# rgoldade/GeometricMultigridPressureSolver

Hardware: AMD Instinct MI355X
Metric: V-cycles/sec (higher is better)
Workload: dtype f32

## Files before the change

### geometricmultigridpressuresolver_amd/csrc/mgps_internal.h

```cpp
#pragma once

#include <cstdint>
#include <cstdlib>
#include <cstddef>
#include <memory>
#include <string>
#include <utility>
#include <vector>

#include "mgps.h"

namespace mgps {

constexpr int kTile = 16;

constexpr int kChunkCells = 1024;
constexpr int kWaveChunkCells = 256;
constexpr int kSegCells = 32;

void *hostBigAlloc(size_t bytes);
void hostBigFree(void *p);
void setHostBigAllocator(void *(*alloc)(size_t), void (*release)(void *));
constexpr size_t kBigBlockBytes = size_t(1) << 20;

// ... 102 lines not shown
                   bool needCoarseSolver);
void setLastGlobalError(const std::string &msg);
const char *lastGlobalError();
int apiException(const mgps_solver *h) noexcept;
extern void (*gSetHandleError)(const mgps_solver *h, const char *msg) noexcept;
#define MGPS_API_CATCH(h) catch (...) { return ::mgps::apiException(h); }

struct GridP {
    int nx, ny, nz;
    const uint8_t *lab;
    const float *wx, *wy, *wz;
    const int32_t *bnd;
    const float *rows;
    int nbnd;
    const uint8_t *bandDiag;
    int ghostLo, ghostHi;
    const int32_t *chunks;
    int nchunks, chunkCells;
    const int32_t *planeBlocks;
    int nplaneBlocks, planeZc;
    int streaming;
    int sweepPath;
    int xlo, xhi;
};
int launchActiveXRange(void *stream, const uint8_t *lab, int nx, size_t cells, int *range);

struct MixScale {
    const float *sigma = nullptr;
    float c1 = 1.f, c2 = 1.f;
};

constexpr int kPlaneRows = 16;
constexpr size_t kPlaneSweepMinPlaneBytes = size_t(4) << 20;
constexpr int kSlabEdgePlanes = kBandMaxDepth + 1;
inline int planeSweepZc(int nx, int ny, int nz)
{
    if ((nx & 3) != 0 || nx < 256 || ny < kPlaneRows) return 0;
    const size_t nbx = (nx + 255) / 256, nby = (ny + kPlaneRows - 1) / kPlaneRows;
    int zc = 32;
    while (zc > 4 && nbx * nby * size_t((nz + zc - 1) / zc) < 1024) zc >>= 1;
    return zc;
}

enum StencilOp { OP_JACOBI = 0, OP_RESIDUAL = 1, OP_APPLY = 2 };

size_t stencilSweptCells(const GridP &g);
int stencilKernelOf(const GridP &g);
// ... 216 lines not shown
```

### geometricmultigridpressuresolver_amd/csrc/mgps_kernels.hip

```cpp
#include <hip/hip_runtime.h>
#include <hip/hip_fp16.h>

#include <algorithm>
#include <cstdlib>
#include <type_traits>

#include "mgps_internal.h"

namespace mgps {

namespace {

typedef float v4f __attribute__((ext_vector_type(4)));
typedef unsigned char v4b __attribute__((ext_vector_type(4)));
__device__ __forceinline__ float4 streamLoad4(const float *p)
{
    const v4f v = __builtin_nontemporal_load(reinterpret_cast<const v4f *>(p));
    return make_float4(v.x, v.y, v.z, v.w);
}
__device__ __forceinline__ uchar4 streamLoad4(const uint8_t *p)
{
    const v4b v = __builtin_nontemporal_load(reinterpret_cast<const v4b *>(p));
    return make_uchar4(v.x, v.y, v.z, v.w);
}
// ... 112 lines not shown
    return (bid % kXcds) * per + bid / kXcds;
}

__device__ __forceinline__ bool listQuad(const int32_t *__restrict__ chunks, int chunkCells, size_t block, size_t &t, unsigned tid)
{
    if (chunkCells == kChunkCells) {
        t = size_t(chunks[block]) * 256 + tid;
        return true;
    }
    int ch;
    if (chunkCells == kWaveChunkCells) {
        ch = chunks[block * 4 + __builtin_amdgcn_readfirstlane(tid >> 6)];
        t = size_t(max(ch, 0)) * kWave + (tid & (kWave - 1));
    } else {
        const int lanes = chunkCells >> 2, shift = __ffs(lanes) - 1;
        ch = chunks[(block << (8 - shift)) + (tid >> shift)];
        t = (size_t(max(ch, 0)) << shift) + (tid & (lanes - 1));
    }
    return ch >= 0;
}
__device__ __forceinline__ bool listQuad(const int32_t *__restrict__ chunks, int chunkCells, size_t block, size_t &t) { return listQuad(chunks, chunkCells, block, t, threadIdx.x); }
__device__ __forceinline__ int listRunMask(const int32_t *chunks, int chunkCells) { return (chunks && chunkCells < kWaveChunkCells) ? (chunkCells >> 2) - 1 : kWave - 1; }

template <int OP, bool DOT, class TX, bool XZERO, bool KEEP>
__device__ __forceinline__ void stencilQuadBody(const GridP &g, TX *__restrict__ out, const TX *__restrict__ x, const float *__restrict__ b, float omega,
                                                unsigned nblocks, const int32_t *__restrict__ chunks, double *__restrict__ dotPartials, const MixScale &ms,
                                                unsigned vblock, unsigned tid, const uint32_t *__restrict__ keep)
{
    constexpr bool kMixed = !std::is_same<TX, float>::value;
    const unsigned nq = unsigned(g.nx) >> 2;
    const size_t rows = size_t(g.ny) * g.nz;
    const size_t totalQuads = size_t(nq) * rows;
    const unsigned block = remapBlock(vblock, nblocks);
    size_t t = size_t(block) * 256 + tid;
    bool valid = true;
    if (chunks) valid = listQuad(chunks, g.chunkCells, block, t, tid);
    valid = valid && t < totalQuads;
    const size_t tt = valid ? t : totalQuads - 1;
    const size_t c = tt << 2;
    const size_t sy = size_t(g.nx), sz = size_t(g.nx) * g.ny, ncells = totalQuads << 2;
    const bool nqPow2 = (nq & (nq - 1u)) == 0u;
    const int i = int((nqPow2 ? (unsigned(tt) & (nq - 1u)) : (totalQuads <= 0xffffffffull ? unsigned(tt) % nq : unsigned(tt % nq))) << 2);

    const float4 zero4 = make_float4(0.f, 0.f, 0.f, 0.f);
    const bool live = i >= g.xlo && i < g.xhi;
    valid = valid && live;
// ... 75 lines not shown
}
#define MGPS_GLOBAL_AS __attribute__((address_space(1)))
__device__ __forceinline__ float4 gLoad4(const float *base, unsigned cell)
{
    const v4f v = *(const MGPS_GLOBAL_AS v4f *)((const MGPS_GLOBAL_AS char *)base + cell * 4u);
    return make_float4(v.x, v.y, v.z, v.w);
}
__device__ __forceinline__ float4 gLoad4nt(const float *base, unsigned cell)
{
    const v4f v = __builtin_nontemporal_load((const MGPS_GLOBAL_AS v4f *)((const MGPS_GLOBAL_AS char *)base + cell * 4u));
    return make_float4(v.x, v.y, v.z, v.w);
}
__device__ __forceinline__ float gLoad1(const float *base, unsigned cell) { return *(const MGPS_GLOBAL_AS float *)((const MGPS_GLOBAL_AS char *)base + cell * 4u); }
__device__ __forceinline__ float2 gLoad2(const float *base, unsigned cell)
{
    typedef float v2f __attribute__((ext_vector_type(2)));
    const v2f v = *(const MGPS_GLOBAL_AS v2f *)((const MGPS_GLOBAL_AS char *)base + cell * 4u);
    return make_float2(v.x, v.y);
}
__device__ __forceinline__ uchar4 gLoadCodes4nt(const uint8_t *base, unsigned cell)
{
    const v4b v = __builtin_nontemporal_load((const MGPS_GLOBAL_AS v4b *)((const MGPS_GLOBAL_AS char *)base + cell));
    return make_uchar4(v.x, v.y, v.z, v.w);
}
__device__ __forceinline__ unsigned gLoadCode1(const uint8_t *base, unsigned cell) { return *((const MGPS_GLOBAL_AS uint8_t *)base + cell); }
__device__ __forceinline__ void gStore4(float *base, unsigned cell, float4 v) { *(MGPS_GLOBAL_AS v4f *)((MGPS_GLOBAL_AS char *)base + cell * 4u) = v4f{v.x, v.y, v.z, v.w}; }
__device__ __forceinline__ void gStore4nt(float *base, unsigned cell, float4 v)
{
    __builtin_nontemporal_store(v4f{v.x, v.y, v.z, v.w}, (MGPS_GLOBAL_AS v4f *)((MGPS_GLOBAL_AS char *)base + cell * 4u));
}
typedef float v2f __attribute__((ext_vector_type(2)));
__device__ __forceinline__ void gStore2(float *base, unsigned cell, float2 v) { *(MGPS_GLOBAL_AS v2f *)((MGPS_GLOBAL_AS char *)base + cell * 4u) = v2f{v.x, v.y}; }
__device__ __forceinline__ void gStore2nt(float *base, unsigned cell, float2 v)
{
    __builtin_nontemporal_store(v2f{v.x, v.y}, (MGPS_GLOBAL_AS v2f *)((MGPS_GLOBAL_AS char *)base + cell * 4u));
}

__device__ __forceinline__ float fromLeftLane(float v) { return __int_as_float(__builtin_amdgcn_update_dpp(0, __float_as_int(v), 0x138, 0xf, 0xf, false)); }
__device__ __forceinline__ float fromRightLane(float v) { return __int_as_float(__builtin_amdgcn_update_dpp(0, __float_as_int(v), 0x130, 0xf, 0xf, false)); }
typedef float v4fu __attribute__((ext_vector_type(4), aligned(4)));
__device__ __forceinline__ float4 gLoad4u(const float *base, unsigned cell)
{
    const v4fu v = *(const MGPS_GLOBAL_AS v4fu *)((const MGPS_GLOBAL_AS char *)base + cell * 4u);
    return make_float4(v.x, v.y, v.z, v.w);
}

// ... 11 lines not shown
    double dotAcc = 0.0;
    __shared__ float plane[2][(kPlaneRows + 2) * kPlanePitch];
    unsigned bid = remapBlock(blockIdx.x, gridDim.x);
    if (blocks) bid = unsigned(blocks[bid]);
    bid = __builtin_amdgcn_readfirstlane(bid);
    const unsigned bx = bid % nbx, by = (bid / nbx) % nby, bz = bid / (nbx * nby);
    const int lane = threadIdx.x & (kWave - 1), ty = threadIdx.x / kWave;
    const int i = int(bx) * 256 + lane * 4, j = int(by) * kPlaneRows + ty;
    const int ic = min(i, g.nx - 4), jc = min(j, g.ny - 1);
    const bool live = ic >= g.xlo && ic < g.xhi;
    const bool valid = i < g.nx && j < g.ny && live;
    const bool ld = live && !XZERO;
    const ptrdiff_t sz = ptrdiff_t(g.nx) * g.ny;
    const int k0 = int(bz) * zc, k1 = min(k0 + zc, g.nz);
    const int kLo = g.ghostLo ? -1 : 0, kHi = g.ghostHi ? g.nz : g.nz - 1;
    const unsigned off = unsigned(jc) * unsigned(g.nx) + unsigned(ic);
    const unsigned offYm = jc > 0 ? off - unsigned(g.nx) : off, offYp = jc < g.ny - 1 ? off + unsigned(g.nx) : off;
    auto planeOf = [&](const float *p, int k) { return scalarBase(p + ptrdiff_t(min(max(k, kLo), kHi)) * sz); };
    const bool rowTop = ty == 0, rowBot = ty == kPlaneRows - 1, colL = lane == 0, colR = lane == kWave - 1;
    const bool useHx = ld && ((colL && ic > 0) || (colR && ic + 4 < g.nx));
    const unsigned offHx = !useHx ? off : (colL ? off - 1u : off + 4u);

    const float4 zero4 = make_float4(0.f, 0.f, 0.f, 0.f);
    const uchar4 ext4 = make_uchar4(MGPS_EXTERIOR_CELL, MGPS_EXTERIOR_CELL, MGPS_EXTERIOR_CELL, MGPS_EXTERIOR_CELL);
    float *const mine0 = plane[0] + (ty + 1) * kPlanePitch + 4 + lane * 4;
    constexpr int kBufFloats = (kPlaneRows + 2) * kPlanePitch;
    *reinterpret_cast<float4 *>(mine0 + kBufFloats) = ld ? gLoad4(planeOf(x, k0 - 1), off) : zero4;
    const float *xk = XZERO ? x : planeOf(x, k0);
    float4 xc = ld ? gLoad4(xk, off) : zero4;
    float4 xp = ld ? gLoad4(planeOf(x, k0 + 1), off) : zero4;
    float4 hy = zero4;
    if (ld && rowTop) hy = gLoad4(xk, offYm);
    if (ld && rowBot) hy = gLoad4(xk, offYp);
    float hx = ld ? gLoad1(xk, offHx) : 0.f;

    int buf = 0;
    for (int k = k0; k < k1; ++k) {
        float *me = mine0 + buf * kBufFloats;
        *reinterpret_cast<float4 *>(me) = xc;
        if (rowTop) *reinterpret_cast<float4 *>(me - kPlanePitch) = hy;
        if (rowBot) *reinterpret_cast<float4 *>(me + kPlanePitch) = hy;
        if (colL) me[-1] = useHx ? hx : 0.f;
        if (colR) me[4] = useHx ? hx : 0.f;
        float4 bc = zero4;
        uchar4 lc = ext4;
        if (live) {
            if (OP != OP_APPLY) bc = gLoad4nt(scalarBase(b + ptrdiff_t(k) * sz), off);
            lc = gLoadCodes4nt(scalarBase(g.lab + ptrdiff_t(k) * sz), off);
        }
        float4 xq = zero4, hyn = hy;
        float hxn = hx;
        if (k + 1 < k1 && ld) {
            const float *xn = planeOf(x, k + 1);
            xq = gLoad4(planeOf(x, k + 2), off);
            if (rowTop) hyn = gLoad4(xn, offYm);
            if (rowBot) hyn = gLoad4(xn, offYp);
            hxn = gLoad1(xn, offHx);
        }
        __syncthreads();
        const float4 ym = *reinterpret_cast<const float4 *>(me - kPlanePitch);
        const float4 yp = *reinterpret_cast<const float4 *>(me + kPlanePitch);
        const float4 xm = *reinterpret_cast<const float4 *>(mine0 + (buf ^ 1) * kBufFloats);
        const float xs[6] = {me[-1], xc.x, xc.y, xc.z, xc.w, me[4]};
        const float yms[4] = {ym.x, ym.y, ym.z, ym.w}, yps[4] = {yp.x, yp.y, yp.z, yp.w};
        const float zms[4] = {xm.x, xm.y, xm.z, xm.w}, zps[4] = {xp.x, xp.y, xp.z, xp.w};
        const float bs[4] = {bc.x, bc.y, bc.z, bc.w};
        const unsigned ls[4] = {lc.x, lc.y, lc.z, lc.w};
        float res[4];
#pragma unroll
        for (int e = 0; e < 4; ++e) {
            const float diag = simpleDiag(ls[e]);
            const float lap = diag * xs[e + 1] - (xs[e] + xs[e + 2] + yms[e] + yps[e] + zms[e] + zps[e]);
            res[e] = simpleCell(ls[e]) ? epilogueRcp<OP>(xs[e + 1], bs[e], lap, simpleRcp(diag), omega) : inactiveValue<OP>(xs[e + 1]);
        }
        if (valid)
            gStore4nt(scalarBase(out + ptrdiff_t(k) * sz), off, make_float4(res[0], res[1], res[2], res[3]));
        if (DOT) {
#pragma unroll
            for (int e = 0; e < 4; ++e)
                if (valid && simpleCell(ls[e])) dotAcc += dotTerm<OP>(xs[e + 1], bs[e], res[e]);
        }
        xc = xp;
        xp = xq;
        hy = hyn;
        hx = hxn;
        buf ^= 1;
    }
    if (DOT) {
        __syncthreads();
// ... 14 lines not shown
    __shared__ float crow[kUpRing][kUpRows * kPlanePitch];
    unsigned bid = remapBlock(blockIdx.x, gridDim.x);
    if (blocks) bid = unsigned(blocks[bid]);
    bid = __builtin_amdgcn_readfirstlane(bid);
    const unsigned bx = bid % nbx, by = (bid / nbx) % nby, bz = bid / (nbx * nby);
    const int lane = threadIdx.x & (kWave - 1), ty = threadIdx.x / kWave;
    const int i = int(bx) * 256 + lane * 4, j = int(by) * kPlaneRows + ty;
    const int ic = min(i, g.nx - 4), jc = min(j, g.ny - 1);
    const bool live = ic >= g.xlo && ic < g.xhi;
    const bool valid = i < g.nx && j < g.ny && live;
    const ptrdiff_t sz = ptrdiff_t(g.nx) * g.ny;
    const int k0 = int(bz) * zc, k1 = min(k0 + zc, g.nz);
    const unsigned off = unsigned(jc) * unsigned(g.nx) + unsigned(ic);
    const unsigned offYm = jc > 0 ? off - unsigned(g.nx) : off, offYp = jc < g.ny - 1 ? off + unsigned(g.nx) : off;
    auto planeOf = [&](const float *p, int k) { return scalarBase(p + ptrdiff_t(min(max(k, 0), g.nz - 1)) * sz); };
    const bool rowTop = ty == 0, rowBot = ty == kPlaneRows - 1, colL = lane == 0, colR = lane == kWave - 1;
    const bool useHx = live && ((colL && ic > 0) || (colR && ic + 4 < g.nx));
    const unsigned offHx = !useHx ? off : (colL ? off - 1u : off + 4u);
    auto opq = [](unsigned v) {
        asm volatile("" : "+v"(v));
        return v;
    };
    const float4 zero4 = make_float4(0.f, 0.f, 0.f, 0.f);
    const uchar4 ext4 = make_uchar4(MGPS_EXTERIOR_CELL, MGPS_EXTERIOR_CELL, MGPS_EXTERIOR_CELL, MGPS_EXTERIOR_CELL);

    const int cnx = g.nx >> 1, cny = g.ny >> 1, cnz = g.nz >> 1;
    const ptrdiff_t csz = ptrdiff_t(cnx) * cny;
    const int tid = threadIdx.x;
    const bool stager = tid < kUpStagers;
    const int sr = tid / kUpQuads, sq = tid - sr * kUpQuads;
    const int mq = min(max(int(bx) * 64 - 1 + sq, 0), (g.nx >> 2) - 1);
    const int crw = min(max(int(by) * (kPlaneRows / 2) - 1 + sr, 0), cny - 1);
    const unsigned cOff1 = unsigned(crw) * unsigned(cnx) + unsigned(2 * mq);
    auto slotOf = [](int P) { return (P + kUpRing) % kUpRing; };
    auto cplane = [&](int P) { return scalarBase(coarse + ptrdiff_t(min(max(P, 0), cnz - 1)) * csz); };
    auto loadC = [&](const float *p) {
        const float2 c12 = gLoad2(p, opq(cOff1));
        return make_float4(gLoad1(p, opq(mq > 0 ? cOff1 - 1u : cOff1)), c12.x, c12.y, gLoad1(p, opq(2 * mq + 2 < cnx ? cOff1 + 2u : cOff1 + 1u)));
    };
    auto stageC = [&](int P, float4 c) {
        *reinterpret_cast<float4 *>(&crow[slotOf(P)][sr * kPlanePitch + 4 * sq]) =
            make_float4(lerpRef(c.x, c.y, 0.75f), lerpRef(c.y, c.z, 0.25f), lerpRef(c.y, c.z, 0.75f), lerpRef(c.z, c.w, 0.25f));
    };
    const int rowBase = 1 - int(by) * (kPlaneRows / 2);
    auto rowsAt = [&](int kk, int jj, int xi, const float *&pa, const float *&pb, float &fy, float &fz) {
        const int Pa = (kk - 1) >> 1;
        const int o = (((jj - 1) >> 1) + rowBase) * kPlanePitch + xi;
        pa = &crow[slotOf(Pa)][o];
        pb = &crow[slotOf(Pa + 1)][o];
        fy = (jj & 1) ? 0.25f : 0.75f;
        fz = (kk & 1) ? 0.25f : 0.75f;
    };
    auto trilerp = [](float a0, float a1, float b0, float b1, float fy, float fz) { return lerpRef(lerpRef(a0, a1, fy), lerpRef(b0, b1, fy), fz); };
    auto corr4 = [&](int kk, int jj, float4 v, uchar4 lc, bool act) {
        const float *pa, *pb;
        float fy, fz;
        rowsAt(kk, jj, 4 + lane * 4, pa, pb, fy, fz);
        const float4 a0 = *reinterpret_cast<const float4 *>(pa), a1 = *reinterpret_cast<const float4 *>(pa + kPlanePitch);
        const float4 ya = make_float4(lerpRef(a0.x, a1.x, fy), lerpRef(a0.y, a1.y, fy), lerpRef(a0.z, a1.z, fy), lerpRef(a0.w, a1.w, fy));
        asm volatile("" ::: "memory");
        const float4 b0 = *reinterpret_cast<const float4 *>(pb), b1 = *reinterpret_cast<const float4 *>(pb + kPlanePitch);
        const float t0 = lerpRef(ya.x, lerpRef(b0.x, b1.x, fy), fz), t1 = lerpRef(ya.y, lerpRef(b0.y, b1.y, fy), fz);
        const float t2 = lerpRef(ya.z, lerpRef(b0.z, b1.z, fy), fz), t3 = lerpRef(ya.w, lerpRef(b0.w, b1.w, fy), fz);
        return make_float4(!act || activeLabel(lc.x) ? v.x + 4.f * t0 : v.x, !act || activeLabel(lc.y) ? v.y + 4.f * t1 : v.y,
                           !act || activeLabel(lc.z) ? v.z + 4.f * t2 : v.z, !act || activeLabel(lc.w) ? v.w + 4.f * t3 : v.w);
    };
    auto corr1 = [&](int kk, int jj, float v) {
        const float *pa, *pb;
        float fy, fz;
        rowsAt(kk, jj, colL ? 3 : 4 + 256, pa, pb, fy, fz);
        return v + 4.f * trilerp(pa[0], pa[kPlanePitch], pb[0], pb[kPlanePitch], fy, fz);
    };

    {
        const float *p0 = cplane((k0 >> 1) - 1), *p1 = cplane(k0 >> 1), *p2 = cplane((k0 >> 1) + 1);
        const float4 c0 = stager ? loadC(p0) : zero4, c1 = stager ? loadC(p1) : zero4, c2 = stager ? loadC(p2) : zero4;
        if (stager) {
            stageC((k0 >> 1) - 1, c0);
            stageC(k0 >> 1, c1);
            stageC((k0 >> 1) + 1, c2);
        }
    }
    float *const mine0 = plane[0] + (ty + 1) * kPlanePitch + 4 + lane * 4;
    constexpr int kBufFloats = (kPlaneRows + 2) * kPlanePitch;
    float4 xm0 = live ? gLoad4(planeOf(x, k0 - 1), off) : zero4;
    const float *xk = planeOf(x, k0);
    float4 xc = live ? gLoad4(xk, off) : zero4;
    float4 xp = live ? gLoad4(planeOf(x, k0 + 1), off) : zero4;
    const uint8_t *lab0 = scalarBase(g.lab + ptrdiff_t(k0) * sz);
    uchar4 lc = live ? gLoadCodes4nt(lab0, off) : ext4;
    uchar4 lcn = live ? gLoadCodes4nt(scalarBase(g.lab + ptrdiff_t(k0 + 1) * sz), off) : ext4;
    float4 hy = zero4;
    if (live && rowTop) hy = gLoad4(xk, offYm);
    if (live && rowBot) hy = gLoad4(xk, offYp);
    float hx = live ? gLoad1(xk, offHx) : 0.f;
    __syncthreads();
    if (live) {
        xm0 = corr4(k0 - 1, j, xm0, lc, false);
        xc = corr4(k0, j, xc, lc, true);
    }
    *reinterpret_cast<float4 *>(mine0 + kBufFloats) = xm0;

    int buf = 0;
    for (int k = k0; k < k1; ++k) {
        float *me = mine0 + buf * kBufFloats;
        if (live) {
            if (rowTop) hy = corr4(k, j - 1, hy, lc, false);
            if (rowBot) hy = corr4(k, j + 1, hy, lc, false);
            if (useHx) hx = corr1(k, j, hx);
            xp = corr4(k + 1, j, xp, lcn, k + 1 < k1);
        }
        *reinterpret_cast<float4 *>(me) = xc;
        if (rowTop) *reinterpret_cast<float4 *>(me - kPlanePitch) = hy;
        if (rowBot) *reinterpret_cast<float4 *>(me + kPlanePitch) = hy;
        if (colL) me[-1] = useHx ? hx : 0.f;
        if (colR) me[4] = useHx ? hx : 0.f;
        float4 bc = zero4;
        uchar4 lcq = ext4;
        const float *bk = scalarBase(b + ptrdiff_t(k) * sz);
        const uint8_t *labq = scalarBase(g.lab + ptrdiff_t(min(k + 2, g.nz - 1)) * sz);
        if (live) {
            bc = gLoad4nt(bk, opq(off));
            if (k + 2 < k1) lcq = gLoadCodes4nt(labq, opq(off));
        }
        float4 xq = zero4, hyn = hy;
        float hxn = hx;
        if (k + 1 < k1 && live) {
            const float *xn = planeOf(x, k + 1);
            xq = gLoad4(planeOf(x, k + 2), opq(off));
            if (rowTop) hyn = gLoad4(xn, opq(offYm));
            if (rowBot) hyn = gLoad4(xn, opq(offYp));
            hxn = gLoad1(xn, opq(offHx));
        }
        const bool stageNext = !(k & 1) && k + 2 < k1;
        const float *pn = cplane((k >> 1) + 2);
        float4 cnext = zero4;
        if (stageNext && stager) cnext = loadC(pn);
        __syncthreads();
        if (stageNext && stager) stageC((k >> 1) + 2, cnext);
        const float4 ym = *reinterpret_cast<const float4 *>(me - kPlanePitch);
        const float4 yp = *reinterpret_cast<const float4 *>(me + kPlanePitch);
        const float4 xm = *reinterpret_cast<const float4 *>(mine0 + (buf ^ 1) * kBufFloats);
        const float xs[6] = {me[-1], xc.x, xc.y, xc.z, xc.w, me[4]};
        const float yms[4] = {ym.x, ym.y, ym.z, ym.w}, yps[4] = {yp.x, yp.y, yp.z, yp.w};
        const float zms[4] = {xm.x, xm.y, xm.z, xm.w}, zps[4] = {xp.x, xp.y, xp.z, xp.w};
        const float bs[4] = {bc.x, bc.y, bc.z, bc.w};
        const unsigned ls[4] = {lc.x, lc.y, lc.z, lc.w};
        float res[4];
#pragma unroll
        for (int e = 0; e < 4; ++e) {
            const float diag = simpleDiag(ls[e]);
            const float lap = diag * xs[e + 1] - (xs[e] + xs[e + 2] + yms[e] + yps[e] + zms[e] + zps[e]);
            res[e] = simpleCell(ls[e]) ? epilogueRcp<OP_JACOBI>(xs[e + 1], bs[e], lap, simpleRcp(diag), omega) : inactiveValue<OP_JACOBI>(xs[e + 1]);
        }
        if (valid) gStore4nt(scalarBase(out + ptrdiff_t(k) * sz), opq(off), make_float4(res[0], res[1], res[2], res[3]));
        xc = xp;
        xp = xq;
        hy = hyn;
        hx = hxn;
        lc = lcn;
        lcn = lcq;
        buf ^= 1;
    }
}

template <bool XF>
__global__ __launch_bounds__(64 * kPlaneRows, 8) void residualZKernel(GridP g, float *__restrict__ rz, const float *__restrict__ x,
                                                                     const float *__restrict__ b, unsigned nbx, unsigned nby, int zc,
                                                                     const int32_t *__restrict__ blocks, const float *__restrict__ rEdge,
                                                                     float *__restrict__ seam)
// ... 22 lines not shown
    {
        const float4 xm = gLoad4(planeOf(x, ks - 1), offL);
        *reinterpret_cast<float4 *>(mine0 + kBufFloats) = keepIf(xm, live);
    }
    const float *xk = planeOf(x, ks);
    float4 xc = gLoad4(xk, offL);
    float4 xp = gLoad4(planeOf(x, ks + 1), offL);
    float4 hy = gLoad4(xk, offHy);
    const bool useHx = live && ((colL && hasL) || (colR && hasR));
    const unsigned offHx = !useHx ? offL : colL ? offL - 1u : offL + 4u;
    float hx = gLoad1(xk, offHx);
    constexpr float w0 = 0.125f, w1 = 0.375f, w2 = 0.375f, w3 = 0.125f;
    float accPrev[4] = {0.f, 0.f, 0.f, 0.f}, accCur[4] = {0.f, 0.f, 0.f, 0.f};
    const unsigned rowS = __builtin_amdgcn_readfirstlane(unsigned(jc));
    const unsigned rowX = rowS * (unsigned(g.nx) >> 1) + bx * 128u, rowSeam = (rowS * (nbx - 1u) + bx) * 8u;
    const bool storeX = i < g.nx && j < g.ny && ic >= g.xlo - 4 && ic < g.xhi + 4;
    const bool seamL = colL && bx > 0, seamR = colR && i + 4 < g.nx;
    const bool seamW = valid && (seamL || seamR);
    auto storeFolded = [&](int K, bool nt) {
        const float4 v = keepIf(make_float4(accPrev[0], accPrev[1], accPrev[2], accPrev[3]), valid);
        const float2 o = make_float2(foldX4(fromLeftLane(v.w), v.x, v.y, v.z), foldX4(v.y, v.z, v.w, fromRightLane(v.x)));
        float *const px = scalarBase(rz + size_t(K) * (sz >> 1));
        if (storeX) {
            const unsigned offX = rowX + 2u * unsigned(lane);
            if (nt) gStore2nt(px, offX, o);
            else gStore2(px, offX, o);
        }
        if (seamW) gStore4(scalarBase(seam + size_t(K) * size_t(g.ny) * size_t(nbx - 1u) * 8u), colL ? rowSeam - 4u : rowSeam, v);
    };
    if (rEdge && k0 == 0 && g.ghostLo) {
        const float4 e = gLoad4(scalarBase(rEdge - ptrdiff_t(sz)), offL);
        accCur[0] = w0 * e.x;
        accCur[1] = w0 * e.y;
        accCur[2] = w0 * e.z;
        accCur[3] = w0 * e.w;
    }
    int buf = 0;
    for (int k = ks; k <= ke; ++k) {
        float *me = mine0 + buf * kBufFloats;
        xc = keepIf(xc, live);
        *reinterpret_cast<float4 *>(me) = xc;
        if (rowTop) *reinterpret_cast<float4 *>(me - kPlanePitch) = keepIf(hy, live);
        if (rowBot) *reinterpret_cast<float4 *>(me + kPlanePitch) = keepIf(hy, live);
        if (colL) me[-1] = useHx ? hx : 0.f;
        if (colR) me[4] = useHx ? hx : 0.f;
        const float *bk = planeOf(b, k);
        const uint8_t *lk = scalarBase(g.lab + size_t(k) * sz);
        const float *xn = planeOf(x, k + 1), *xq2 = planeOf(x, k + 2);
        const float4 bc = gLoad4nt(bk, offL);
        const uchar4 lc = gLoadCodes4nt(lk, offL);
        const float hxn = gLoad1(xn, offHx);
        float4 hyn = hy;
        if (rowTop || rowBot) hyn = gLoad4(xn, offHy);
        const float4 xq = gLoad4(xq2, offL);
        __syncthreads();
        const float4 ym = *reinterpret_cast<const float4 *>(me - kPlanePitch);
        const float4 yp = *reinterpret_cast<const float4 *>(me + kPlanePitch);
        const float4 xm = *reinterpret_cast<const float4 *>(mine0 + (buf ^ 1) * kBufFloats);
        const float xs[6] = {me[-1], xc.x, xc.y, xc.z, xc.w, me[4]};
        const float yms[4] = {ym.x, ym.y, ym.z, ym.w}, yps[4] = {yp.x, yp.y, yp.z, yp.w};
        const float zms[4] = {xm.x, xm.y, xm.z, xm.w}, zps[4] = {xp.x, xp.y, xp.z, xp.w};
        const float bs[4] = {bc.x, bc.y, bc.z, bc.w};
        const unsigned ls[4] = {lc.x, lc.y, lc.z, lc.w};
        float res[4];
#pragma unroll
        for (int e = 0; e < 4; ++e) {
            const float diag = simpleDiag(ls[e]);
            const float lap = diag * xs[e + 1] - (xs[e] + xs[e + 2] + yms[e] + yps[e] + zms[e] + zps[e]);
            res[e] = simpleCell(ls[e]) ? epilogueRcp<OP_RESIDUAL>(xs[e + 1], bs[e], lap, simpleRcp(diag), 0.f) : inactiveValue<OP_RESIDUAL>(xs[e + 1]);
        }
        if (k & 1) {
#pragma unroll
            for (int e = 0; e < 4; ++e) {
                accPrev[e] = accCur[e] + w2 * res[e];
                accCur[e] = w0 * res[e];
            }
        } else {
#pragma unroll
            for (int e = 0; e < 4; ++e) {
                accPrev[e] += w3 * res[e];
                accCur[e] += w1 * res[e];
            }
            if (XF) {
                if (k >= k0 + 2) storeFolded((k >> 1) - 1, true);
            } else if (valid && k >= k0 + 2) {
// ... 1592 lines not shown
                lo = min(lo, int(4 * qi) + __ffs(any) - 1);
                hi = max(hi, int(4 * qi) + 31 - __clz(any));
            }
        }
    }
#pragma unroll
    for (int off = kWave / 2; off > 0; off >>= 1) {
        lo = min(lo, __shfl_down(lo, off));
        hi = max(hi, __shfl_down(hi, off));
    }
    if ((threadIdx.x & (kWave - 1)) == 0 && hi >= 0) {
        atomicMin(range, lo);
        atomicMax(range + 1, hi);
    }
}
int launchActiveXRange(void *stream, const uint8_t *lab, int nx, size_t cells, int *range)
{
    if (cells == 0 || (nx & 3) != 0 || nx < 16) return 0;
    const unsigned nb = unsigned(std::min<size_t>((cells / 16 + 255) / 256, 256 * 32));
    activeXRangeKernel<<<std::max(nb, 1u), 256, 0, static_cast<hipStream_t>(stream)>>>(lab, nx, cells, range);
    return int(hipGetLastError());
}

static unsigned sweepBlocks(const GridP &g, bool skipInactive, int *path)
{
    const size_t n = size_t(g.nx) * g.ny * g.nz;
    const int forced = forcedStencil(g);
    const int zc = g.planeZc;
    const bool planeWins = size_t(g.nx) * g.ny * sizeof(float) > kPlaneSweepMinPlaneBytes;
    if (zc && (forced == 2 || (forced == 0 && planeWins))) {
        *path = 0;
        const unsigned nbx = (g.nx + 255) / 256, nby = (g.ny + kPlaneRows - 1) / kPlaneRows, nbz = (g.nz + zc - 1) / zc;
        return (skipInactive && g.planeBlocks) ? unsigned(g.nplaneBlocks) : nbx * nby * nbz;
    }
    if ((g.nx & 3) == 0) {
        *path = 1;
        return (skipInactive && g.chunks) ? unsigned(g.nchunks) / unsigned(kChunkCells / g.chunkCells) : blocksFor(n >> 2, 256);
    }
    *path = 2;
    return blocksFor(n, 256);
}

int stencilKernelOf(const GridP &g)
{
    int path = 0;
    (void)sweepBlocks(g, true, &path);
// ... 362 lines not shown
}
std::vector<int32_t> planeBlockEdges(const GridP &g, const std::vector<uint8_t> &flags)
{
    const int zc = g.planeZc > 0 ? g.planeZc : 1;
    const size_t layer = size_t((g.nx + 255) / 256) * size_t((g.ny + kPlaneRows - 1) / kPlaneRows), nbz = size_t((g.nz + zc - 1) / zc);
    std::vector<int32_t> edges;
    for (size_t bid = 0; bid < flags.size() && bid < layer * nbz; ++bid) {
        if (flags[bid]) continue;
        const size_t bz = bid / layer;
        if (bz > 0 && flags[bid - layer]) edges.push_back(int32_t(2 * bid));
        if (bz + 1 < nbz && flags[bid + layer]) edges.push_back(int32_t(2 * bid + 1));
    }
    return edges;
}
int launchResidualEdgePlanes(void *stream, const GridP &g, float *r, const float *x, const float *b)
{
    const size_t sz = size_t(g.nx) * g.ny;
    for (int side = 0; side < 2; ++side) {
        if (!(side == 0 ? g.ghostLo : g.ghostHi)) continue;
        const int k = side == 0 ? 0 : g.nz - 1;
        GridP p = g;
        p.nz = 1;
        p.lab = g.lab + size_t(k) * sz;
        p.ghostLo = (k > 0 || g.ghostLo) ? 1 : 0;
        p.ghostHi = (k < g.nz - 1 || g.ghostHi) ? 1 : 0;
        p.chunks = nullptr;
        p.nchunks = 0;
        p.planeBlocks = nullptr;
        p.nplaneBlocks = 0;
        p.planeZc = 0;
        p.sweepPath = 1;
        p.nbnd = 0;
        p.streaming = 0;
        const int e = launchStencil(stream, OP_RESIDUAL, p, r + size_t(k) * sz, x + size_t(k) * sz, b + size_t(k) * sz, 0.f, true);
        if (e) return e;
    }
    if (g.nbnd > 0) {
        const unsigned nb = blocksFor(size_t(g.nbnd), 256);
        boundaryOpKernel<OP_RESIDUAL><<<nb, 256, 0, static_cast<hipStream_t>(stream)>>>(g, r, x, b, 0.f, nb);
    }
    return int(hipGetLastError());
}
bool residualRestrictXFolds(const GridP &fine) { return fine.nbnd == 0; }
static size_t rzxGridFloats(const GridP &fine) { return (size_t(fine.nx) * fine.ny * fine.nz / 4 + 3) & ~size_t(3); }
size_t rzxFloats(const GridP &fine) { return rzxGridFloats(fine) + size_t(fine.nz / 2) * fine.ny * size_t((fine.nx + 255) / 256 - 1) * 8; }
int launchResidualZ(void *stream, const GridP &fine, float *rz, const float *x, const float *b, const int32_t *edges, int nedges, const float *rEdge, bool xfold)
// ... 956 lines not shown
```

### geometricmultigridpressuresolver_amd/csrc/mgps_solver.hip

```cpp
#include <hip/hip_runtime.h>

#include <dlfcn.h>

#include <algorithm>
#include <chrono>
#include <cmath>
#include <cstdio>
#include <cstring>
#include <functional>
#include <limits>
#include <string>
#include <atomic>
#include <mutex>
#include <thread>
#include <unordered_map>
#include <map>
#include <memory>
#include <vector>

#include "mgps_internal.h"

using namespace mgps;

namespace {
// ... 20 lines not shown
    int32_t *tileBndStart = nullptr;
    int z0 = 0, z1 = 0;
    int32_t *bandPlane[4] = {nullptr, nullptr, nullptr, nullptr};
    int nbandPlane[4] = {0, 0, 0, 0};
    float *packBuf[4] = {nullptr, nullptr, nullptr, nullptr};
    int32_t *chunks = nullptr, *planeBlocks = nullptr;
    int edgeChunks = 0, edgePlaneBlocks = 0;
    BandBoxesDev bandBoxes;
    uint8_t *planeFlags = nullptr;
    int32_t *rzEdges = nullptr;
    int nrzEdges = 0;
    float *rz = nullptr;
    uint8_t *snapTile = nullptr;
    uint32_t *keepBits = nullptr;
    struct BoxHalo {
        int32_t *sendIdx[2] = {nullptr, nullptr}, *recvIdx[2] = {nullptr, nullptr};
        int nsend[2] = {0, 0}, nrecv[2] = {0, 0};
        float *sendBuf[2] = {nullptr, nullptr}, *recvBuf[2] = {nullptr, nullptr};
    } halo;
    bool boxForm = false;
    bool hasBandPlanes = false;
    GridP gBox{};
    float *extRows = nullptr;
    int elo = 0;
};

}

struct mgps_solver {
    mgps_hierarchy *hier = nullptr;
    std::vector<mgps_hierarchy *> retiredHier;
    mgps_options opt{};
    bool useGS = false;
    int device = 0;
    hipStream_t stream = nullptr;
    std::vector<DevLevel> lv;
    float *w[3] = {nullptr, nullptr, nullptr};
    bool weightsBorrowed = false;
    int cn = 0;
    float *cinv = nullptr, *cvec = nullptr;
    std::shared_ptr<void> cinvShared;
    int32_t *ccells = nullptr;
    bool tailOfSlabRun = false;
    double *partials = nullptr, *resultDev = nullptr, *resultHost = nullptr;
    double *dotPartials = nullptr;
    double *cg64[4] = {nullptr, nullptr, nullptr, nullptr};
// ... 293 lines not shown
        }
        (void)cacheFree(L.tileBndStart);
        for (int q = 0; q < 4; ++q) {
            (void)cacheFree(L.bandPlane[q]);
            (void)cacheFree(L.packBuf[q]);
        }
        (void)cacheFree(L.chunks);
        (void)cacheFree(L.planeBlocks);
        for (int q = 0; q < 2; ++q) {
            (void)cacheFree(L.halo.sendIdx[q]);
            (void)cacheFree(L.halo.recvIdx[q]);
            (void)cacheFree(L.halo.sendBuf[q]);
            (void)cacheFree(L.halo.recvBuf[q]);
        }
        (void)cacheFree(L.extRows);
        (void)cacheFree(L.bandBoxes.info);
        (void)cacheFree(L.bandBoxes.list);
        (void)cacheFree(L.planeFlags);
        (void)cacheFree(L.keepBits);
        (void)cacheFree(L.snapTile);
        (void)cacheFree(L.rz);
        (void)cacheFree(L.rzEdges);
        (void)cacheFree(L.bandBoxes.general);
    }
    for (int a = 0; a < 3 && !h->weightsBorrowed; ++a) (void)cacheFree(h->w[a]);
    if (!h->cinvShared) (void)cacheFree(h->cinv);
    (void)cacheFree(h->cvec);
    (void)cacheFree(h->ccells);
    (void)cacheFree(h->partials);
    (void)cacheFree(h->resultDev);
    (void)cacheFree(h->dotPartials);
    (void)cacheFree(h->cgScal);
    (void)cacheFree(h->mixX);
    (void)cacheFree(h->mixTmp);
    (void)cacheFree(h->mixR);
    (void)cacheFree(h->mixSigma);
    (void)cacheFree(h->mixMax);
    for (double *g64 : h->cg64)
        if (g64) (void)cacheFree(g64 - size_t(h->lv[0].d.nx) * h->lv[0].d.ny);
    if (h->resultHost) (void)hipHostFree(h->resultHost);
    if (!h->lv.empty()) {
        for (int q = 0; q < 4; ++q) gridFree(h, h->pcg[q], h->lv[0].d);
        gridFree(h, h->dinv, h->lv[0].d);
    }
    for (void *p : {(void *)h->encCellList, (void *)h->encOffsets, (void *)h->encChunks, (void *)h->encCompChunk, (void *)h->encPartials, (void *)h->encSum, (void *)h->encCount})
        (void)cacheFree(p);
// ... 1565 lines not shown
    if (hipHostMalloc(reinterpret_cast<void **>(&h->resultHost), sizeof(double)) != hipSuccess)
        return failH(h, MGPS_ERR_ALLOC, "pinned allocation failed");
    static const bool rangeSkip = [] {
        const char *e = getenv("MGPS_X_RANGE");
        return !(e && e[0] == '0');
    }();
    const size_t nlv = h->lv.size();
    std::vector<int> range(2 * nlv);
    int *rangeDev = nullptr;
    for (size_t l = 0; l < nlv; ++l) {
        range[2 * l] = h->lv[l].g.nx;
        range[2 * l + 1] = -1;
        h->lv[l].g.xlo = 0;
        h->lv[l].g.xhi = h->lv[l].g.nx;
    }
    if (rangeSkip && nlv > 0) {
        MGPS_TRY(devAlloc(h, &rangeDev, 2 * nlv, false));
        MGPS_HIP(h, hipMemcpyAsync(rangeDev, range.data(), range.size() * sizeof(int), hipMemcpyHostToDevice, nullptr));
        for (size_t l = 0; l < nlv; ++l) {
            const GridP &g = h->lv[l].g;
            if (g.lab && (g.nx & 3) == 0) MGPS_LAUNCH(h, launchActiveXRange(nullptr, g.lab, g.nx, size_t(g.nx) * g.ny * g.nz, rangeDev + 2 * l));
        }
        MGPS_HIP(h, hipMemcpyAsync(range.data(), rangeDev, range.size() * sizeof(int), hipMemcpyDeviceToHost, nullptr));
    }
    MGPS_HIP(h, hipDeviceSynchronize());
    if (rangeDev) {
        (void)cacheFree(rangeDev);
        for (size_t l = 0; l < nlv; ++l)
            if (range[2 * l + 1] >= range[2 * l]) {
                h->lv[l].g.xlo = range[2 * l] & ~3;
                h->lv[l].g.xhi = (range[2 * l + 1] | 3) + 1;
            }
    }
    return MGPS_OK;
}

struct PinnedCache {
    std::mutex guard;
    std::vector<std::pair<size_t, void *>> free;
    std::unordered_map<void *, size_t> size;
    size_t cached = 0;
    size_t cap = [] {
        const char *e = getenv("MGPS_PINNED_CACHE_MB");
        return size_t(e ? std::max(0, atoi(e)) : 4096) << 20;
    }();
};
// ... 2161 lines not shown
    case 6: src = L.pure[0], n = size_t(L.npure[0]); break;
    case 7: src = L.pure[1], n = size_t(L.npure[1]); break;
    case 8: src = L.mixed[0], n = size_t(L.nmixed[0]); break;
    case 9: src = L.mixed[1], n = size_t(L.nmixed[1]); break;
    case 10: src = L.tileBndStart, n = size_t(nt) + 1; break;
    case 11: src = L.bandBoxes.info, n = size_t(kBoxInfoInts) * size_t(L.bandBoxes.ngroups); break;
    case 12: src = L.bandBoxes.list, n = L.bandBoxes.listCount; break;
    case 13: src = L.bandBoxes.general, n = L.bandBoxes.generalInts; break;
    case 14: {
        if (level != 0 || h->opt.enclosed_liquid != 1)
            return failH(h, MGPS_ERR_INVALID_ARGUMENT, "mgps_level_array: array 14 exists on level 0 with options.enclosed_liquid only");
        *count = int64_t(L.d.cells());
        if (!out) return MGPS_OK;
        int32_t *rank = nullptr;
        MGPS_TRY(devAlloc(h, &rank, L.d.cells(), false));
        int rc = MGPS_OK;
        if (hipMemsetAsync(rank, 0xff, L.d.cells() * sizeof(int32_t), h->stream) != hipSuccess ||
            launchEnclosedRanks(h->stream, rank, h->encCellList, h->encChunks, h->encNChunks) != 0 || hipStreamSynchronize(h->stream) != hipSuccess ||
            hipMemcpy(out, rank, L.d.cells() * sizeof(int32_t), hipMemcpyDeviceToHost) != hipSuccess)
            rc = failH(h, MGPS_ERR_HIP, "mgps_level_array: enclosed-component ranks");
        (void)cacheFree(rank);
        return rc;
    }
    default: return failH(h, MGPS_ERR_INVALID_ARGUMENT, "mgps_level_array: unknown array");
    }
    *count = int64_t(n);
    if (out && n) {
        MGPS_HIP(h, hipStreamSynchronize(h->stream));
        MGPS_HIP(h, hipMemcpy(out, src, n * elem, hipMemcpyDeviceToHost));
    }
    return MGPS_OK;
}
MGPS_API_CATCH(h)
int mgps_distributed_levels(const mgps_solver *h) { return h ? h->distLevels : 0; }
int mgps_ghost_planes(const mgps_solver *h) { return h ? h->ghost : 1; }
int mgps_residual_restrict_fused(const mgps_solver *h, int level, int *fused)
try {
    if (!h || !fused || level < 0 || level >= int(h->lv.size())) return MGPS_ERR_INVALID_ARGUMENT;
    *fused = residualRestrictFuses(h, level) ? 1 : 0;
    return MGPS_OK;
}
MGPS_API_CATCH(h)
int mgps_residual_restrict_xfolded(const mgps_solver *h, int level, int *xfolded)
try {
    if (!h || !xfolded || level < 0 || level >= int(h->lv.size())) return MGPS_ERR_INVALID_ARGUMENT;
    *xfolded = residualRestrictXFolded(h, level) ? 1 : 0;
// ... 548 lines not shown
```

### geometricmultigridpressuresolver_amd/solver.py

```python
import ctypes as C

import numpy as np
import torch

from . import _lib
from ._lib import Options, PcgStats, check, lib

PCG_OUTCOMES = {0: "converged", 1: "rhs_zero", 2: "already_converged", 3: "max_iterations"}


def _pcg_stats(st):
    return {
        "outcome": PCG_OUTCOMES.get(st.outcome, st.outcome),
        "iterations": st.iterations,
        "rel_residual": st.rel_residual,
        "rel_residual_recomputed": st.rel_residual_recomputed,
        "rhs_norm2": st.rhs_norm2,
        "solve_ms": st.solve_ms,
    }


def _check_pcg(status, handle, st):
    try:
        check(status, handle)
# ... 186 lines not shown
        if getattr(self, "h", None):
            lib().mgps_destroy(self.h)
            self.h = None

    def __del__(self):
        try:
            self.close()
        except Exception:
            pass

    def use_torch_stream(self):
        s = torch.cuda.current_stream(self.device).cuda_stream
        check(lib().mgps_set_stream(self.h, C.c_void_p(s)), self.h)

    def synchronize(self):
        check(lib().mgps_synchronize(self.h), self.h)

    def hierarchy(self):
        return Hierarchy(_borrowed=lib().mgps_get_hierarchy(self.h))

    LEVEL_ARRAYS = {"codes": (0, np.uint8), "band": (1, np.int32), "band_diag": (2, np.uint8), "rows": (3, np.float32), "chunks": (4, np.int32),
                    "plane_blocks": (5, np.int32), "pure_even": (6, np.int32), "pure_odd": (7, np.int32), "mixed_even": (8, np.int32),
                    "mixed_odd": (9, np.int32), "tile_bnd_start": (10, np.int32), "box_info": (11, np.int32), "box_list": (12, np.uint32),
                    "box_general": (13, np.int32)}

    def level_array(self, level, name):
        which, dt = self.LEVEL_ARRAYS[name]
        n = C.c_int64()
        check(lib().mgps_level_array(self.h, int(level), which, None, C.byref(n)), self.h)
        out = np.empty(n.value, dtype=dt)
        if n.value:
            check(lib().mgps_level_array(self.h, int(level), which, _p(out), C.byref(n)), self.h)
        return out

    def level_shape(self, level):
        d = (C.c_int * 3)()
        check(lib().mgps_level_dims(self.h, level, d), self.h)
        return (d[2], d[1], d[0])

    def new_grid(self, level=0):
        return torch.zeros(self.level_shape(level), dtype=torch.float32, device=self.device)

    def to_device(self, a, level=0):
        t = torch.from_numpy(_np_f32(a)).to(self.device)
        assert tuple(t.shape) == self.level_shape(level)
        return t

# ... 187 lines not shown
```

Measured before the change: 122.6.

## Skip label-code loads for all-interior quads using a per-tile plain bitmask

Adds a setup pass that records, per 4-cell quad, whether all cell codes are zero, packed into a 64-bit word per 256-cell row tile. The plane-sweep smoother, interpolation-correction and residual-restrict kernels read this word through the scalar constant path, expand it to per-lane flags with inverse ballot, and skip the per-quad label load when the quad is plain. The aim is to cut byte-code memory traffic in bandwidth-bound sweeps. In exchange it adds scalar loads per plane, extra setup kernels and device memory, and the path is disabled for distributed or ghosted levels.

```diff
diff --git a/geometricmultigridpressuresolver_amd/csrc/mgps_internal.h b/geometricmultigridpressuresolver_amd/csrc/mgps_internal.h
--- a/geometricmultigridpressuresolver_amd/csrc/mgps_internal.h
+++ b/geometricmultigridpressuresolver_amd/csrc/mgps_internal.h
@@ -148,7 +148,11 @@
     int streaming;
     int sweepPath;
     int xlo, xhi;
-};
+    const uint32_t *plainQ;
+    const unsigned long long *plainT;
+};
+inline size_t plainQuadWords(size_t cells) { return ((cells / 4 + 63) / 64) * 2; }
+int launchPlainQuads(void *stream, const uint8_t *lab, int nx, int ny, int nz, uint32_t *plainQ, unsigned long long *plainT);
 int launchActiveXRange(void *stream, const uint8_t *lab, int nx, size_t cells, int *range);
 
 struct MixScale {
diff --git a/geometricmultigridpressuresolver_amd/csrc/mgps_kernels.hip b/geometricmultigridpressuresolver_amd/csrc/mgps_kernels.hip
--- a/geometricmultigridpressuresolver_amd/csrc/mgps_kernels.hip
+++ b/geometricmultigridpressuresolver_amd/csrc/mgps_kernels.hip
@@ -158,6 +158,10 @@
 __device__ __forceinline__ bool listQuad(const int32_t *__restrict__ chunks, int chunkCells, size_t block, size_t &t) { return listQuad(chunks, chunkCells, block, t, threadIdx.x); }
 __device__ __forceinline__ int listRunMask(const int32_t *chunks, int chunkCells) { return (chunks && chunkCells < kWaveChunkCells) ? (chunkCells >> 2) - 1 : kWave - 1; }
 
+#define MGPS_CONST_AS __attribute__((address_space(4)))
+__device__ __forceinline__ unsigned long long plainWord64(const void *base, size_t idx) { return *((const MGPS_CONST_AS unsigned long long *)base + idx); }
+__device__ __forceinline__ bool plainLane(unsigned long long w) { return __builtin_amdgcn_inverse_ballot_w64(w); }
+
 template <int OP, bool DOT, class TX, bool XZERO, bool KEEP>
 __device__ __forceinline__ void stencilQuadBody(const GridP &g, TX *__restrict__ out, const TX *__restrict__ x, const float *__restrict__ b, float omega,
                                                 unsigned nblocks, const int32_t *__restrict__ chunks, double *__restrict__ dotPartials, const MixScale &ms,
@@ -279,6 +283,14 @@
 {
     const v4b v = __builtin_nontemporal_load((const MGPS_GLOBAL_AS v4b *)((const MGPS_GLOBAL_AS char *)base + cell));
     return make_uchar4(v.x, v.y, v.z, v.w);
+}
+__device__ __forceinline__ unsigned gLoadCodesWnt(const uint8_t *base, unsigned cell) { return __builtin_nontemporal_load((const MGPS_GLOBAL_AS unsigned *)((const MGPS_GLOBAL_AS char *)base + cell)); }
+__device__ __forceinline__ uchar4 codes4(unsigned w) { return make_uchar4(w & 255u, (w >> 8) & 255u, (w >> 16) & 255u, w >> 24); }
+__device__ __forceinline__ unsigned laneHere()
+{
+    unsigned z = 0u;
+    asm volatile("" : "+s"(z));
+    return __builtin_amdgcn_mbcnt_hi(~0u, __builtin_amdgcn_mbcnt_lo(~0u, z));
 }
 __device__ __forceinline__ unsigned gLoadCode1(const uint8_t *base, unsigned cell) { return *((const MGPS_GLOBAL_AS uint8_t *)base + cell); }
 __device__ __forceinline__ void gStore4(float *base, unsigned cell, float4 v) { *(MGPS_GLOBAL_AS v4f *)((MGPS_GLOBAL_AS char *)base + cell * 4u) = v4f{v.x, v.y, v.z, v.w}; }
@@ -336,7 +348,10 @@
     const unsigned offHx = !useHx ? off : (colL ? off - 1u : off + 4u);
 
     const float4 zero4 = make_float4(0.f, 0.f, 0.f, 0.f);
-    const uchar4 ext4 = make_uchar4(MGPS_EXTERIOR_CELL, MGPS_EXTERIOR_CELL, MGPS_EXTERIOR_CELL, MGPS_EXTERIOR_CELL);
+    constexpr unsigned extW = 0x01010101u * unsigned(MGPS_EXTERIOR_CELL);
+    const unsigned long long *const pt = g.plainT;
+    const size_t wRow = size_t(__builtin_amdgcn_readfirstlane(unsigned(jc))) * nbx + bx, wPlane = size_t(g.ny) * nbx;
+    unsigned long long pw = pt ? plainWord64(pt, size_t(k0) * wPlane + wRow) : 0ull;
     float *const mine0 = plane[0] + (ty + 1) * kPlanePitch + 4 + lane * 4;
     constexpr int kBufFloats = (kPlaneRows + 2) * kPlanePitch;
     *reinterpret_cast<float4 *>(mine0 + kBufFloats) = ld ? gLoad4(planeOf(x, k0 - 1), off) : zero4;
@@ -357,11 +372,13 @@
         if (colL) me[-1] = useHx ? hx : 0.f;
         if (colR) me[4] = useHx ? hx : 0.f;
         float4 bc = zero4;
-        uchar4 lc = ext4;
+        unsigned lcw = extW;
         if (live) {
             if (OP != OP_APPLY) bc = gLoad4nt(scalarBase(b + ptrdiff_t(k) * sz), off);
-            lc = gLoadCodes4nt(scalarBase(g.lab + ptrdiff_t(k) * sz), off);
-        }
+            lcw = 0u;
+            if (!plainLane(pw)) lcw = gLoadCodesWnt(scalarBase(g.lab + ptrdiff_t(k) * sz), off);
+        }
+        if (pt) pw = plainWord64(pt, size_t(min(k + 1, g.nz - 1)) * wPlane + wRow);
         float4 xq = zero4, hyn = hy;
         float hxn = hx;
         if (k + 1 < k1 && ld) {
@@ -379,6 +396,7 @@
         const float yms[4] = {ym.x, ym.y, ym.z, ym.w}, yps[4] = {yp.x, yp.y, yp.z, yp.w};
         const float zms[4] = {xm.x, xm.y, xm.z, xm.w}, zps[4] = {xp.x, xp.y, xp.z, xp.w};
         const float bs[4] = {bc.x, bc.y, bc.z, bc.w};
+        const uchar4 lc = codes4(lcw);
         const unsigned ls[4] = {lc.x, lc.y, lc.z, lc.w};
         float res[4];
 #pragma unroll
@@ -439,7 +457,6 @@
         return v;
     };
     const float4 zero4 = make_float4(0.f, 0.f, 0.f, 0.f);
-    const uchar4 ext4 = make_uchar4(MGPS_EXTERIOR_CELL, MGPS_EXTERIOR_CELL, MGPS_EXTERIOR_CELL, MGPS_EXTERIOR_CELL);
 
     const int cnx = g.nx >> 1, cny = g.ny >> 1, cnz = g.nz >> 1;
     const ptrdiff_t csz = ptrdiff_t(cnx) * cny;
@@ -469,7 +486,8 @@
         fz = (kk & 1) ? 0.25f : 0.75f;
     };
     auto trilerp = [](float a0, float a1, float b0, float b1, float fy, float fz) { return lerpRef(lerpRef(a0, a1, fy), lerpRef(b0, b1, fy), fz); };
-    auto corr4 = [&](int kk, int jj, float4 v, uchar4 lc, bool act) {
+    auto corr4 = [&](int kk, int jj, float4 v, unsigned lcw, bool act) {
+        const uchar4 lc = codes4(lcw);
         const float *pa, *pb;
         float fy, fz;
         rowsAt(kk, jj, 4 + lane * 4, pa, pb, fy, fz);
@@ -504,9 +522,16 @@
     const float *xk = planeOf(x, k0);
     float4 xc = live ? gLoad4(xk, off) : zero4;
     float4 xp = live ? gLoad4(planeOf(x, k0 + 1), off) : zero4;
+    const unsigned long long *const pt = g.plainT;
+    const size_t wRow = size_t(__builtin_amdgcn_readfirstlane(unsigned(jc))) * nbx + bx, wPlane = size_t(g.ny) * nbx;
+    auto plainAt = [&](int kk) { return pt ? plainWord64(pt, size_t(min(kk, g.nz - 1)) * wPlane + wRow) : 0ull; };
+    const unsigned long long pw0 = plainAt(k0), pw1 = plainAt(k0 + 1);
+    unsigned long long pw = plainAt(k0 + 2);
+    constexpr unsigned extW = 0x01010101u * unsigned(MGPS_EXTERIOR_CELL);
     const uint8_t *lab0 = scalarBase(g.lab + ptrdiff_t(k0) * sz);
-    uchar4 lc = live ? gLoadCodes4nt(lab0, off) : ext4;
-    uchar4 lcn = live ? gLoadCodes4nt(scalarBase(g.lab + ptrdiff_t(k0 + 1) * sz), off) : ext4;
+    unsigned lc = live ? 0u : extW, lcn = lc;
+    if (live && !plainLane(pw0)) lc = gLoadCodesWnt(lab0, off);
+    if (live && !plainLane(pw1)) lcn = gLoadCodesWnt(scalarBase(g.lab + ptrdiff_t(k0 + 1) * sz), off);
     float4 hy = zero4;
     if (live && rowTop) hy = gLoad4(xk, offYm);
     if (live && rowBot) hy = gLoad4(xk, offYp);
@@ -533,13 +558,17 @@
         if (colL) me[-1] = useHx ? hx : 0.f;
         if (colR) me[4] = useHx ? hx : 0.f;
         float4 bc = zero4;
-        uchar4 lcq = ext4;
+        unsigned lcq = extW;
         const float *bk = scalarBase(b + ptrdiff_t(k) * sz);
         const uint8_t *labq = scalarBase(g.lab + ptrdiff_t(min(k + 2, g.nz - 1)) * sz);
         if (live) {
             bc = gLoad4nt(bk, opq(off));
-            if (k + 2 < k1) lcq = gLoadCodes4nt(labq, opq(off));
-        }
+            if (k + 2 < k1) {
+                lcq = 0u;
+                if (!plainLane(pw)) lcq = gLoadCodesWnt(labq, opq(off));
+            }
+        }
+        pw = plainAt(k + 3);
         float4 xq = zero4, hyn = hy;
         float hxn = hx;
         if (k + 1 < k1 && live) {
@@ -562,7 +591,8 @@
         const float yms[4] = {ym.x, ym.y, ym.z, ym.w}, yps[4] = {yp.x, yp.y, yp.z, yp.w};
         const float zms[4] = {xm.x, xm.y, xm.z, xm.w}, zps[4] = {xp.x, xp.y, xp.z, xp.w};
         const float bs[4] = {bc.x, bc.y, bc.z, bc.w};
-        const unsigned ls[4] = {lc.x, lc.y, lc.z, lc.w};
+        const uchar4 lc4 = codes4(lc);
+        const unsigned ls[4] = {lc4.x, lc4.y, lc4.z, lc4.w};
         float res[4];
 #pragma unroll
         for (int e = 0; e < 4; ++e) {
@@ -631,7 +661,7 @@
         const float2 o = make_float2(foldX4(fromLeftLane(v.w), v.x, v.y, v.z), foldX4(v.y, v.z, v.w, fromRightLane(v.x)));
         float *const px = scalarBase(rz + size_t(K) * (sz >> 1));
         if (storeX) {
-            const unsigned offX = rowX + 2u * unsigned(lane);
+            const unsigned offX = rowX + 2u * laneHere();
             if (nt) gStore2nt(px, offX, o);
             else gStore2(px, offX, o);
         }
@@ -644,6 +674,9 @@
         accCur[2] = w0 * e.z;
         accCur[3] = w0 * e.w;
     }
+    const unsigned long long *const pt = g.plainT;
+    const size_t wRow = size_t(rowS) * nbx + bx, wPlane = size_t(g.ny) * nbx;
+    unsigned long long pw = pt ? plainWord64(pt, size_t(ks) * wPlane + wRow) : 0ull;
     int buf = 0;
     for (int k = ks; k <= ke; ++k) {
         float *me = mine0 + buf * kBufFloats;
@@ -656,8 +689,10 @@
         const float *bk = planeOf(b, k);
         const uint8_t *lk = scalarBase(g.lab + size_t(k) * sz);
         const float *xn = planeOf(x, k + 1), *xq2 = planeOf(x, k + 2);
+        unsigned lcw = 0u;
+        if (!plainLane(pw)) lcw = gLoadCodesWnt(lk, offL);
+        if (pt) pw = plainWord64(pt, size_t(min(k + 1, g.nz - 1)) * wPlane + wRow);
         const float4 bc = gLoad4nt(bk, offL);
-        const uchar4 lc = gLoadCodes4nt(lk, offL);
         const float hxn = gLoad1(xn, offHx);
         float4 hyn = hy;
         if (rowTop || rowBot) hyn = gLoad4(xn, offHy);
@@ -670,6 +705,7 @@
         const float yms[4] = {ym.x, ym.y, ym.z, ym.w}, yps[4] = {yp.x, yp.y, yp.z, yp.w};
         const float zms[4] = {xm.x, xm.y, xm.z, xm.w}, zps[4] = {xp.x, xp.y, xp.z, xp.w};
         const float bs[4] = {bc.x, bc.y, bc.z, bc.w};
+        const uchar4 lc = codes4(lcw);
         const unsigned ls[4] = {lc.x, lc.y, lc.z, lc.w};
         float res[4];
 #pragma unroll
@@ -2308,6 +2344,47 @@
     return int(hipGetLastError());
 }
 
+__global__ __launch_bounds__(256) void plainQuadsKernel(const uint8_t *__restrict__ lab, size_t quads, uint32_t *__restrict__ plainQ)
+{
+    const unsigned *w = reinterpret_cast<const unsigned *>(lab);
+    const size_t groups = (quads + kWave - 1) / kWave, waves = size_t(gridDim.x) * (blockDim.x / kWave);
+    const unsigned lane = threadIdx.x & (kWave - 1);
+    for (size_t grp = size_t(blockIdx.x) * (blockDim.x / kWave) + threadIdx.x / kWave; grp < groups; grp += waves) {
+        const size_t q = grp * kWave + lane;
+        const unsigned v = q < quads ? __builtin_nontemporal_load(w + q) : 0x01010101u * unsigned(MGPS_EXTERIOR_CELL);
+        const unsigned long long plain = __ballot(v == 0u);
+        if (lane < 2) plainQ[2 * grp + lane] = unsigned(plain >> (32 * lane));
+    }
+}
+__global__ __launch_bounds__(256) void plainTilesKernel(const uint32_t *__restrict__ plainQ, size_t words, unsigned nq, unsigned nbx, size_t rows,
+                                                        unsigned long long *__restrict__ plainT)
+{
+    const size_t t = size_t(blockIdx.x) * blockDim.x + threadIdx.x;
+    if (t >= rows * nbx) return;
+    const size_t row = t / nbx;
+    const unsigned tile = unsigned(t - row * nbx), left = nq - tile * 64u;
+    const size_t q0 = row * nq + size_t(tile) * 64u, w0 = q0 >> 5;
+    const unsigned sh = unsigned(q0) & 31u;
+    const unsigned long long a = plainQ[w0], b = w0 + 1 < words ? plainQ[w0 + 1] : 0u, c = w0 + 2 < words ? plainQ[w0 + 2] : 0u;
+    unsigned long long v = ((a | (b << 32)) >> sh) | (sh ? c << (64u - sh) : 0ull);
+    if (left < 64u) v &= (1ull << left) - 1ull;
+    plainT[t] = v;
+}
+int launchPlainQuads(void *stream, const uint8_t *lab, int nx, int ny, int nz, uint32_t *plainQ, unsigned long long *plainT)
+{
+    const size_t cells = size_t(nx) * ny * nz, quads = cells >> 2;
+    if (cells == 0 || (nx & 3) != 0) return int(hipErrorInvalidValue);
+    hipStream_t s = static_cast<hipStream_t>(stream);
+    const size_t groups = (quads + kWave - 1) / kWave;
+    plainQuadsKernel<<<unsigned(std::min<size_t>((groups + 3) / 4, 256 * 64)), 256, 0, s>>>(lab, quads, plainQ);
+    if (plainT) {
+        const unsigned nbx = unsigned(nx + 255) / 256u;
+        const size_t rows = size_t(ny) * nz;
+        plainTilesKernel<<<blocksFor(rows * nbx, 256), 256, 0, s>>>(plainQ, plainQuadWords(cells), unsigned(nx) >> 2, nbx, rows, plainT);
+    }
+    return int(hipGetLastError());
+}
+
 static unsigned sweepBlocks(const GridP &g, bool skipInactive, int *path)
 {
     const size_t n = size_t(g.nx) * g.ny * g.nz;
@@ -2716,6 +2793,8 @@
         GridP p = g;
         p.nz = 1;
         p.lab = g.lab + size_t(k) * sz;
+        p.plainQ = nullptr;
+        p.plainT = nullptr;
         p.ghostLo = (k > 0 || g.ghostLo) ? 1 : 0;
         p.ghostHi = (k < g.nz - 1 || g.ghostHi) ? 1 : 0;
         p.chunks = nullptr;
diff --git a/geometricmultigridpressuresolver_amd/csrc/mgps_solver.hip b/geometricmultigridpressuresolver_amd/csrc/mgps_solver.hip
--- a/geometricmultigridpressuresolver_amd/csrc/mgps_solver.hip
+++ b/geometricmultigridpressuresolver_amd/csrc/mgps_solver.hip
@@ -66,6 +66,8 @@
     bool hasBandPlanes = false;
     GridP gBox{};
     float *extRows = nullptr;
+    uint32_t *plainQ = nullptr;
+    unsigned long long *plainT = nullptr;
     int elo = 0;
 };
 
@@ -405,6 +407,8 @@
         (void)cacheFree(L.rz);
         (void)cacheFree(L.rzEdges);
         (void)cacheFree(L.bandBoxes.general);
+        (void)cacheFree(L.plainQ);
+        (void)cacheFree(L.plainT);
     }
     for (int a = 0; a < 3 && !h->weightsBorrowed; ++a) (void)cacheFree(h->w[a]);
     if (!h->cinvShared) (void)cacheFree(h->cinv);
@@ -2016,6 +2020,21 @@
             if (g.lab && (g.nx & 3) == 0) MGPS_LAUNCH(h, launchActiveXRange(nullptr, g.lab, g.nx, size_t(g.nx) * g.ny * g.nz, rangeDev + 2 * l));
         }
         MGPS_HIP(h, hipMemcpyAsync(range.data(), rangeDev, range.size() * sizeof(int), hipMemcpyDeviceToHost, nullptr));
+    }
+    static const bool plainQuads = [] {
+        const char *e = getenv("MGPS_PLAIN_QUADS");
+        return !(e && e[0] == '0');
+    }();
+    for (size_t l = 0; l < nlv && plainQuads && !h->dist; ++l) {
+        DevLevel &L = h->lv[l];
+        const GridP &g = L.g;
+        if (!g.lab || (g.nx & 3) != 0 || g.ghostLo || g.ghostHi || g.planeZc <= 0 || L.plainQ) continue;
+        const size_t cells = size_t(g.nx) * g.ny * g.nz;
+        MGPS_TRY(devAlloc(h, &L.plainQ, plainQuadWords(cells), false));
+        MGPS_TRY(devAlloc(h, &L.plainT, size_t(g.ny) * g.nz * size_t((g.nx + 255) / 256), false));
+        MGPS_LAUNCH(h, launchPlainQuads(nullptr, g.lab, g.nx, g.ny, g.nz, L.plainQ, L.plainT));
+        L.g.plainQ = L.plainQ;
+        L.g.plainT = L.plainT;
     }
     MGPS_HIP(h, hipDeviceSynchronize());
     if (rangeDev) {
@@ -4223,6 +4242,8 @@
         (void)cacheFree(rank);
         return rc;
     }
+    case 15: src = L.g.plainQ, n = L.g.plainQ ? (L.d.cells() / 4 + 31) / 32 : 0; break;
+    case 16: src = L.g.plainT, n = L.g.plainT ? size_t(L.d.ny) * L.d.nz * size_t((L.d.nx + 255) / 256) : 0, elem = 8; break;
     default: return failH(h, MGPS_ERR_INVALID_ARGUMENT, "mgps_level_array: unknown array");
     }
     *count = int64_t(n);
diff --git a/geometricmultigridpressuresolver_amd/solver.py b/geometricmultigridpressuresolver_amd/solver.py
--- a/geometricmultigridpressuresolver_amd/solver.py
+++ b/geometricmultigridpressuresolver_amd/solver.py
@@ -232,7 +232,7 @@
     LEVEL_ARRAYS = {"codes": (0, np.uint8), "band": (1, np.int32), "band_diag": (2, np.uint8), "rows": (3, np.float32), "chunks": (4, np.int32),
                     "plane_blocks": (5, np.int32), "pure_even": (6, np.int32), "pure_odd": (7, np.int32), "mixed_even": (8, np.int32),
                     "mixed_odd": (9, np.int32), "tile_bnd_start": (10, np.int32), "box_info": (11, np.int32), "box_list": (12, np.uint32),
-                    "box_general": (13, np.int32)}
+                    "box_general": (13, np.int32), "plain_quads": (15, np.uint32), "plain_tiles": (16, np.uint64)}
 
     def level_array(self, level, name):
         which, dt = self.LEVEL_ARRAYS[name]
```

Result: faster. 125.6, median of 6 (+2.5%).
